# arkworks-rs/accumulation

Hardware: AMD Instinct MI355X
Metric: MSM throughput (point-scalar pairs/sec) at 2^20 Pallas (higher is better)
Workload: dtype u32; 1 GPU; 2^20-pair pallas MSM per GPU (north_star size; scalars uniform in [0, r), G_i = k_i*G), key resident + precomputed window multiples; pairs_per_gpu=1048576, curve=pallas, precomputed_key=True, parallelism=point-sharded x1, window_bits=20, pipeline=bucket-per-lane (k_prep_local_t + k_accum_bpl; skewed scalars re-run chunked), window_widths=9 x 20 + 4 x 19 bits = 256 (MsmGeom::n_narrow), msms_in_flight=3, full=False

## Files before the change

accumulation_amd/csrc/kern_fr.hip:

```cpp
#include "launch.h"
#include "vec_kernels.h"
#include "prep_kernels.h"

#include <algorithm>
#include <cmath>
#include <atomic>
#include <cstdlib>
#include <cstring>

namespace amsm {

static inline u32 cdiv_(u32 a, u32 b) { return (a + b - 1) / b; }
static u32 stream_grid(u32 n) {
  constexpr u32 per_cu = 64;
  static const u32 cus = [] {
    int dev = 0;
    hipDeviceProp_t prop;
    if (hipGetDevice(&dev) != hipSuccess || hipGetDeviceProperties(&prop, dev) != hipSuccess) return 256u;
    return (u32)std::max(1, prop.multiProcessorCount);
  }();
  return std::max(1u, std::min(cdiv_(n, 256), cus * per_cu));
}

void launch_bounds(hipStream_t st, const void* keys_sorted, bool keys16, u32* vals_sorted, MsmGeom g, u32* start,
                   u32* items) {
  if (keys16)
    hipLaunchKernelGGL((k_bounds<uint16_t>), dim3(cdiv_(g.B, 256)), dim3(256), 0, st, (const uint16_t*)keys_sorted,
                       vals_sorted, g, start, items);
  else
    hipLaunchKernelGGL((k_bounds<u32>), dim3(cdiv_(g.B, 256)), dim3(256), 0, st, (const u32*)keys_sorted, vals_sorted,
                       g, start, items);
}

constexpr u32 PREP_MAX_P = 4096;
static PrepGeom prep_geom(const MsmGeom& g) {
  PrepGeom pg;
  pg.SH = 4;
  while (((g.B + (1u << pg.SH) - 1u) >> pg.SH) > 512u && pg.SH < 10u) pg.SH++;
  while (((g.B + (1u << pg.SH) - 1u) >> pg.SH) > PREP_MAX_P) pg.SH++;
  pg.P = (g.B + (1u << pg.SH) - 1u) >> pg.SH;
  pg.SPB = g.S <= 16u ? 512u : 256u;
  unsigned long long max_idx = (unsigned long long)g.base_off + g.n - 1ull +
                               (g.precomp ? (unsigned long long)(g.W - 1u) * g.table_stride : 0ull);
  if (g.idx_rel_bits) max_idx = ((unsigned long long)(g.W - 1u) << g.idx_rel_bits) | ((1ull << g.idx_rel_bits) - 1ull);
  pg.IB = 1;
  while ((max_idx >> pg.IB) != 0ull) pg.IB++;
  while (pg.IB + pg.SH > 31u && pg.SH > 0u && ((g.B + (1u << (pg.SH - 1)) - 1u) >> (pg.SH - 1)) <= PREP_MAX_P) pg.SH--;
  pg.P = (g.B + (1u << pg.SH) - 1u) >> pg.SH;
  const u32 budget_words = 37888u, fixed_words = 2u * (1u << pg.SH) + 1024u;
  pg.CAP = budget_words > fixed_words + 4096u ? budget_words - fixed_words : 0u;
  pg.HEAVY = std::max<u32>(4u * (g.E / pg.P + 1u), 1u << 17);
  pg.FIX = 0;
  return pg;
}
static size_t prep_heavy_words(const MsmGeom& g) { return (size_t)g.B + 4096 + 64; }
size_t prep_small_words(const MsmGeom& g) { return 4 * (PREP_MAX_P + 1) + 1 + 3 * prep_heavy_words(g) + PREP_MAX_HEAVY; }
static size_t prep_local_lds(const PrepGeom& pg) { return (2 * (size_t)(1u << pg.SH) + 1024 + pg.CAP) * sizeof(u32); }
constexpr size_t PREP_LDS_LIMIT = 160 * 1024;
static std::atomic<unsigned long long> prep_local_attr_devices{0};
static void prep_local_attr() {
  int dev = 0;
  if (hipGetDevice(&dev) != hipSuccess || dev < 0 || dev >= 64) dev = 63;
  const unsigned long long bit = 1ull << dev;
  if (dev != 63 && (prep_local_attr_devices.load(std::memory_order_acquire) & bit)) return;
  (void)hipFuncSetAttribute((const void*)k_prep_local, hipFuncAttributeMaxDynamicSharedMemorySize, 152 * 1024);
  prep_local_attr_devices.fetch_or(bit, std::memory_order_release);
}
static size_t prep_scatter_lds(const MsmGeom& g, const PrepGeom& pg) {
  const size_t cap = (size_t)pg.SPB * g.S;
  return (3 * (size_t)pg.P + cap) * sizeof(u32) + cap * sizeof(uint16_t);
}
bool prep_supported(const MsmGeom& g) {
  if (g.n == 0 || g.S > 32u) return false;
  PrepGeom pg = prep_geom(g);
  return pg.SH <= 12u && pg.IB + pg.SH <= 31u && prep_scatter_lds(g, pg) <= PREP_LDS_LIMIT &&
         prep_local_lds(pg) <= PREP_LDS_LIMIT && (pg.P + 256) * sizeof(u32) <= 64 * 1024;
}

constexpr u32 BPL_LOCAL_FIXED_WORDS = 3u * BPL_NB + 2u * BPL_BINS + 2u * BPL_GROUPS + 2u;
constexpr u32 BPL_LOCAL_BUDGET_WORDS = 40960u;
static PrepGeom prep_bpl_geom(const MsmGeom& g) {
  PrepGeom pg;
  pg.SH = 10;
  pg.P = g.B >> pg.SH;
  pg.SPB = g.S <= 16u ? 512u : 256u;
  unsigned long long max_idx = (unsigned long long)g.base_off + g.n - 1ull +
                               (g.precomp ? (unsigned long long)(g.W - 1u) * g.table_stride : 0ull);
  if (g.idx_rel_bits) max_idx = ((unsigned long long)(g.W - 1u) << g.idx_rel_bits) | ((1ull << g.idx_rel_bits) - 1ull);
  pg.IB = 1;
  while ((max_idx >> pg.IB) != 0ull) pg.IB++;
  pg.CAP = BPL_LOCAL_BUDGET_WORDS - BPL_LOCAL_FIXED_WORDS;
  pg.HEAVY = 0xffffffffu;
  const unsigned long long per = std::max<unsigned long long>(((unsigned long long)g.E + pg.P - 1) / std::max(1u, pg.P), g.part_max);
  pg.FIX = (u32)std::min<unsigned long long>(pg.CAP, (per + per / 4ull + 2048ull + 15ull) & ~15ull);
  return pg;
}
size_t prep_bpl_part_entries(const MsmGeom& g) {
  PrepGeom pg = prep_bpl_geom(g);
  return std::max<size_t>(g.E, pg.FIX ? (size_t)pg.P * pg.FIX : 0);
}
static size_t prep_bpl_local_lds(const PrepGeom& pg) { return (size_t)(BPL_LOCAL_FIXED_WORDS + pg.CAP) * sizeof(u32); }
static size_t prep_bpl_scatter_lds(const MsmGeom& g, const PrepGeom& pg) {
  const size_t cap = (size_t)pg.SPB * g.S;
  return (3 * (size_t)pg.P + 2 * cap) * sizeof(u32) + cap * sizeof(uint16_t);
}
u32 prep_bpl_partitions(const MsmGeom& g) { return g.B >> 10; }
u32 prep_bpl_groups_per_partition() { return BPL_GROUPS; }
u32 prep_bpl_stride(const MsmGeom& g) {
  const u32 P = std::max(1u, prep_bpl_partitions(g));
  const unsigned long long per = std::max<unsigned long long>(((unsigned long long)g.E + P - 1) / P, g.part_max);
  return (u32)((per + per / 4ull + 4096ull + 1023ull) & ~1023ull);
}
bool prep_bpl_supported(const MsmGeom& g) {
  if (g.S > 32u || g.n == 0 || g.n_sets != g.groups * sets_per_group(g)) return false;
  if (g.B < (1u << 16) || (g.B & 1023u) || (g.B >> 10) > PREP_MAX_P || ((g.B >> 10) & 3u)) return false;
  PrepGeom pg = prep_bpl_geom(g);
  if (pg.IB > 30u) return false;
  if ((unsigned long long)g.E / pg.P + 1024ull > pg.CAP) return false;
  if (g.part_max && (unsigned long long)g.part_max + 5ull * (unsigned long long)std::sqrt((double)g.part_max) > pg.CAP) return false;
  return prep_bpl_scatter_lds(g, pg) <= PREP_LDS_LIMIT && prep_bpl_local_lds(pg) <= PREP_LDS_LIMIT &&
         (unsigned long long)pg.P * prep_bpl_stride(g) < (1ull << 31);
}
static std::atomic<unsigned long long> prep_bpl_attr_devices{0};
template <class KS>
static void prep_bpl_attr(KS scatter_kernel) {
  int dev = 0;
  if (hipGetDevice(&dev) != hipSuccess || dev < 0 || dev >= 64) dev = 63;
  const unsigned long long bit = 1ull << dev;
  (void)hipFuncSetAttribute((const void*)scatter_kernel, hipFuncAttributeMaxDynamicSharedMemorySize, (int)PREP_LDS_LIMIT);
  if (dev != 63 && (prep_bpl_attr_devices.load(std::memory_order_acquire) & bit)) return;
  static_assert((BPL_LOCAL_BUDGET_WORDS) * sizeof(u32) <= PREP_LDS_LIMIT, "k_prep_local_t's LDS must fit a workgroup");
  (void)hipFuncSetAttribute((const void*)k_prep_local_t, hipFuncAttributeMaxDynamicSharedMemorySize, (int)PREP_LDS_LIMIT);
  prep_bpl_attr_devices.fetch_or(bit, std::memory_order_release);
}

constexpr u32 bps_local_fixed_words(u32 nbp) { return 4u * nbp + 1024u + BPL_BINS + 2u * BPS_GROUPS + 2u; }
constexpr u32 BPS_LOCAL_BUDGET_WORDS = 37888u;
static PrepGeom prep_bps_geom(const MsmGeom& g, u32 log2_l) {
  PrepGeom pg;
  pg.SH = 10u - log2_l;
  pg.P = g.B >> pg.SH;
  pg.SPB = g.S <= 16u ? 512u : 256u;
  unsigned long long max_idx = (unsigned long long)g.base_off + g.n - 1ull +
                               (g.precomp ? (unsigned long long)(g.W - 1u) * g.table_stride : 0ull);
  if (g.idx_rel_bits) max_idx = ((unsigned long long)(g.W - 1u) << g.idx_rel_bits) | ((1ull << g.idx_rel_bits) - 1ull);
  pg.IB = 1;
  while ((max_idx >> pg.IB) != 0ull) pg.IB++;
  pg.CAP = BPS_LOCAL_BUDGET_WORDS - bps_local_fixed_words(1u << pg.SH);
  pg.HEAVY = 0xffffffffu;
  const unsigned long long per = ((unsigned long long)g.E + pg.P - 1) / std::max(1u, pg.P);
  pg.FIX = (u32)std::min<unsigned long long>(pg.CAP, (per + per / 2ull + 1024ull + 15ull) & ~15ull);
  return pg;
}
size_t prep_bps_part_entries(const MsmGeom& g, u32 log2_l) {
  PrepGeom pg = prep_bps_geom(g, log2_l);
  return std::max<size_t>(g.E, pg.FIX ? (size_t)pg.P * pg.FIX : 0);
}
static size_t prep_bps_local_lds(const PrepGeom& pg) {
  return (size_t)(bps_local_fixed_words(1u << pg.SH) + pg.CAP) * sizeof(u32);
}
u32 prep_bps_partitions(const MsmGeom& g, u32 log2_l) { return g.B >> (10u - log2_l); }
u32 prep_bps_stride(const MsmGeom& g, u32 log2_l) {
  const u32 P = std::max(1u, prep_bps_partitions(g, log2_l));
  const unsigned long long per = ((unsigned long long)g.E + P - 1) / P;
  return (u32)((per + per / 2ull + 4096ull + 1023ull) & ~1023ull);
}
int prep_bps_choose(const MsmGeom& g) {
  if (!g.precomp || g.n == 0 || g.S > 32u || g.B < 64u || (g.B & (g.B - 1u))) return -1;
  unsigned long long want = 128;
  while (want * 24576ull < g.E) want <<= 1;
  for (int l = 0; l <= 6; l++) {
    if ((10 - l) < 0 || (g.B >> (10 - l)) == 0) continue;
    const unsigned long long P = g.B >> (10 - l);
    if (P < want && l < 6) continue;
    if (P > PREP_MAX_P || (P & 1ull)) return -1;
    MsmGeom g2 = g;
    PrepGeom pg = prep_bps_geom(g2, (u32)l);
    if (pg.IB + pg.SH > 31u) return -1;
    if ((unsigned long long)g.E / P + 1024ull > pg.CAP) return -1;
    if (prep_scatter_lds(g, pg) > PREP_LDS_LIMIT || prep_bps_local_lds(pg) > PREP_LDS_LIMIT) return -1;
    if (P * (unsigned long long)prep_bps_stride(g, (u32)l) >= (1ull << 31)) return -1;
    return l;
  }
  return -1;
}
constexpr size_t PREP_BPS_ZERO_BYTES = (((16 + 4 * (PREP_MAX_P + 1) + 1) * sizeof(u32)) + 255) & ~(size_t)255;
u32 prep_bps_small_block_words() { return (u32)(PREP_BPS_ZERO_BYTES / sizeof(u32)); }
static std::atomic<unsigned long long> prep_bps_attr_devices{0};
static void prep_bps_attr() {
  int dev = 0;
  if (hipGetDevice(&dev) != hipSuccess || dev < 0 || dev >= 64) dev = 63;
  const unsigned long long bit = 1ull << dev;
  if (dev != 63 && (prep_bps_attr_devices.load(std::memory_order_acquire) & bit)) return;
  static_assert(BPS_LOCAL_BUDGET_WORDS * sizeof(u32) <= 152 * 1024, "k_prep_local_s's LDS must fit its attribute");
  (void)hipFuncSetAttribute((const void*)k_prep_local_s, hipFuncAttributeMaxDynamicSharedMemorySize, 152 * 1024);
  (void)hipFuncSetAttribute((const void*)k_prep_local_s_batch, hipFuncAttributeMaxDynamicSharedMemorySize, 152 * 1024);
  prep_bps_attr_devices.fetch_or(bit, std::memory_order_release);
}

__global__ void k_mirror_flags(const u32* __restrict__ flags, u32* __restrict__ host_mirror) {
  if (threadIdx.x < 2u) host_mirror[threadIdx.x] = flags[threadIdx.x];
}
void launch_mirror_flags(hipStream_t st, const u32* flags, u32* host_mirror) {
  hipLaunchKernelGGL(k_mirror_flags, dim3(1), dim3(64), 0, st, flags, host_mirror);
}
void launch_vec_fill(hipStream_t st, u32* out, const u32 v[8], u32 n) {
  hipLaunchKernelGGL(k_vec_fill, dim3(cdiv_(n, 256)), dim3(256), 0, st, out, make_uint4(v[0], v[1], v[2], v[3]),
                     make_uint4(v[4], v[5], v[6], v[7]), n);
}

void launch_tv_probe(hipStream_t st, const u32* scalars, u32 n, u32* out16, const u32 one[8]) {
  static_assert(TV_PROBE_WORDS == TV_WORDS && TV_EXC_SLOTS == TV_EXC_MAX && TV_ONES_SAMPLE_COUNT == TV_ONES_SAMPLES,
                "launch.h mirrors vec_kernels.h");
  const u32 blocks = std::max(1u, std::min(512u, (n + 1023u) / 1024u));
  TvOne o;
  memcpy(o.w, one, 32);
  hipLaunchKernelGGL(k_tv_probe, dim3(blocks), dim3(256), 0, st, scalars, n, out16, o);
}

#define AMSM_FR_LAUNCHERS(FR)                                                                                        \
  template <>                                                                                                        \
  int launch_prep<FR>(hipStream_t st, const u32* scalars, int mont, MsmGeom g, const PrepBuffers& b) {               \
    PrepGeom pg = prep_geom(g);                                                                                      \
    prep_local_attr();                                                                                               \
    u32* part_total = b.d_small;                                                                                     \
    u32* part_start = b.d_small + (PREP_MAX_P + 1);                                                                  \
    u32* part_cursor = b.d_small + 2 * (PREP_MAX_P + 1);                                                             \
    u32* part_items = b.d_small + 3 * (PREP_MAX_P + 1);                                                              \
    PrepHeavy hv;                                                                                                    \
    hv.n = b.d_small + 4 * (PREP_MAX_P + 1);                                                                         \
    hv.cnt = hv.n + 1;                                                          \
    hv.ids = hv.cnt + prep_heavy_words(g);                                                                           \
    hv.cur = hv.ids + PREP_MAX_HEAVY;                                                                                \
    hv.end = hv.cur + prep_heavy_words(g);                                                                           \
     \
     \
                                                                      \
    {                                                                                                                \
      size_t zero_bytes = (16 + 4 * (PREP_MAX_P + 1) + 1 + prep_heavy_words(g)) * sizeof(u32);                       \
      zero_bytes = (zero_bytes + 255) & ~(size_t)255;                                                                \
      if (b.err != b.d_small - 16) return -1;                                                                        \
      if (hipMemsetAsync(b.err, 0, zero_bytes, st) != hipSuccess) return -1;                                         \
    }                                                                                                                \
    u32 blocks = cdiv_(g.n, pg.SPB);                                                                                 \
    size_t lds_scatter = prep_scatter_lds(g, pg);                                                                    \
    if (lds_scatter > 64 * 1024) {                 \
      if (g.S <= 16u)                                                                                                \
        (void)hipFuncSetAttribute((const void*)k_prep_scatter<FR, 16, 1>, hipFuncAttributeMaxDynamicSharedMemorySize, \
                                  (int)PREP_LDS_LIMIT);                                                              \
      else                                                                                                           \
        (void)hipFuncSetAttribute((const void*)k_prep_scatter<FR, 32, 1>, hipFuncAttributeMaxDynamicSharedMemorySize, \
                                  (int)PREP_LDS_LIMIT);                                                              \
    }                                                                                                                \
    {                      \
      PrepGeom ph = pg;                                                                                              \
      ph.SPB = 1024;                                                                                                 \
      hipLaunchKernelGGL((k_prep_hist<FR>), dim3(cdiv_(g.n, 1024)), dim3(1024), pg.P * sizeof(u32), st, scalars,      \
                         mont, g, ph, part_total, b.err);                                                            \
    }                                                                                                                \
    hipLaunchKernelGGL(k_prep_scan, dim3(1), dim3(1024), 0, st, part_total, part_start, pg.P, pg.HEAVY, hv);         \
    if (g.S <= 16u)                                                                                                  \
      hipLaunchKernelGGL((k_prep_scatter<FR, 16, 1>), dim3(blocks), dim3(512), lds_scatter, st, scalars, mont, g, pg, \
                         part_start, part_cursor, b.part);                                                           \
    else                                                                                                             \
      hipLaunchKernelGGL((k_prep_scatter<FR, 32, 1>), dim3(blocks), dim3(256), lds_scatter, st, scalars, mont, g, pg, \
                         part_start, part_cursor, b.part);                                                           \
    const size_t lds_heavy = 2 * (size_t)(1u << pg.SH) * sizeof(u32);                                                \
    if (pg.HEAVY != 0xffffffffu)                                                                                     \
      hipLaunchKernelGGL(k_prep_heavy_count, dim3(PREP_HEAVY_GRID), dim3(256), lds_heavy, st, part_start, b.part, pg, hv); \
    hipLaunchKernelGGL(k_prep_local, dim3(pg.P), dim3(1024), prep_local_lds(pg), st,                                 \
                       part_start, b.part, g, pg, b.vals_sorted, b.start, b.items, b.item_off, part_items, hv);      \
    if (pg.HEAVY != 0xffffffffu)                                                                                     \
      hipLaunchKernelGGL(k_prep_heavy_place, dim3(PREP_HEAVY_GRID), dim3(256), lds_heavy, st, part_start, b.part, g, pg, hv, \
                         b.vals_sorted);                                                                             \
    hipLaunchKernelGGL(k_prep_offsets, dim3(cdiv_(g.B, 256)), dim3(256), (pg.P + 256) * sizeof(u32), st, part_start, \
                       part_items, pg, g, b.start, b.items, b.item_off, b.vals_sorted);                              \
    return 0;                                                                                                        \
  }                                                                                                                  \
  template <>                                                                                                        \
  int launch_prep_bps<FR>(hipStream_t st, const u32* scalars, int mont, MsmGeom g, u32 log2_l, const PrepBplBuffers& b) { \
    PrepGeom pg = prep_bps_geom(g, log2_l);                                                                          \
    u32* part_total = b.d_small;                                                                                     \
    u32* part_start = b.d_small + (PREP_MAX_P + 1);                                                                  \
    u32* part_cursor = b.d_small + 2 * (PREP_MAX_P + 1);                                                             \
    PrepHeavy hv;                                                                                                    \
    hv.n = b.d_small + 4 * (PREP_MAX_P + 1);                                                                         \
    hv.cnt = hv.n + 1;                                                                                               \
    hv.ids = hv.cnt + 64;                                                                                            \
    hv.cur = hv.end = hv.ids;                                                                                        \
    {                                                                                                                \
      size_t zero_bytes = (16 + 4 * (PREP_MAX_P + 1) + 1) * sizeof(u32);                                             \
      zero_bytes = (zero_bytes + 255) & ~(size_t)255;                                                                \
      if (b.err != b.d_small - 16) return -1;                                                                        \
      if (hipMemsetAsync(b.err, 0, zero_bytes, st) != hipSuccess) return -1;                                         \
    }                                                                                                                \
    prep_bps_attr();                                                                                                 \
    if (!pg.FIX) {                                                                                                   \
      PrepGeom ph = pg;                                                                                              \
      ph.SPB = 1024;                                                                                                 \
      hipLaunchKernelGGL((k_prep_hist<FR>), dim3(cdiv_(g.n, 1024)), dim3(1024), pg.P * sizeof(u32), st, scalars,      \
                         mont, g, ph, part_total, b.err);                                                            \
      hipLaunchKernelGGL(k_prep_scan, dim3(1), dim3(1024), 0, st, part_total, part_start, pg.P, pg.HEAVY, hv);       \
    }                                                                                                                \
    const size_t lds_scatter = prep_scatter_lds(g, pg);                                                              \
    if (g.S <= 16u) {                                                                                                \
      if (lds_scatter > 64 * 1024)                                                                                   \
        (void)hipFuncSetAttribute((const void*)k_prep_scatter<FR, 16, 1>, hipFuncAttributeMaxDynamicSharedMemorySize, \
                                  (int)PREP_LDS_LIMIT);                                                              \
      hipLaunchKernelGGL((k_prep_scatter<FR, 16, 1>), dim3(cdiv_(g.n, pg.SPB)), dim3(512), lds_scatter, st, scalars, \
                         mont, g, pg, part_start, part_cursor, b.part, b.err);                                       \
    } else {                                                                                                         \
      if (lds_scatter > 64 * 1024)                                                                                   \
        (void)hipFuncSetAttribute((const void*)k_prep_scatter<FR, 32, 1>, hipFuncAttributeMaxDynamicSharedMemorySize, \
                                  (int)PREP_LDS_LIMIT);                                                              \
      hipLaunchKernelGGL((k_prep_scatter<FR, 32, 1>), dim3(cdiv_(g.n, pg.SPB)), dim3(256), lds_scatter, st, scalars, \
                         mont, g, pg, part_start, part_cursor, b.part, b.err);                                       \
    }                                                                                                                \
    hipLaunchKernelGGL(k_prep_local_s, dim3(pg.P), dim3(1024), prep_bps_local_lds(pg), st,                           \
                       pg.FIX ? part_cursor : part_start, b.part, g, pg,                                             \
                       prep_bps_stride(g, log2_l), log2_l, b.ents_t, (BplGroup*)b.grp, b.order, b.err);              \
    return 0;                                                                                                        \
  }                                                                                                                  \
  template <>                                                                                                        \
  int launch_prep_bps_batch<FR>(hipStream_t st, const u32* const* scalars, u32 nv, int mont, MsmGeom g, u32 log2_l,   \
                                const BpsBatchBuffers& b) {                                                          \
    PrepGeom pg = prep_bps_geom(g, log2_l);                                                                          \
    const u32 stride = prep_bps_stride(g, log2_l);                                                                   \
                                  \
     \
     \
    if (nv < 1u || nv > (u32)PREP_BPS_BATCH || !pg.FIX || g.S > 16u || b.small_stride < prep_bps_small_block_words() || \
        (b.small_stride & 63u) || b.part_stride < prep_bps_part_entries(g, log2_l) ||                                \
        (unsigned long long)b.ents_stride < (unsigned long long)pg.P * stride || b.grp_stride < pg.P * BPS_GROUPS ||  \
        b.order_stride < g.B)                                                                                        \
      return -1;                                                                                                     \
    BpsBatchScalars sc;                                                                                              \
    for (u32 v = 0; v < (u32)PREP_BPS_BATCH; v++) sc.scalars[v] = scalars[v < nv ? v : 0u];                          \
    u32* part_start0 = b.small + 16 + (PREP_MAX_P + 1);                                                              \
    u32* part_cursor0 = b.small + 16 + 2 * (PREP_MAX_P + 1);                                                         \
                                                         \
    if (hipMemsetAsync(b.small, 0, (size_t)nv * b.small_stride * sizeof(u32), st) != hipSuccess) return -1;          \
    prep_bps_attr();                                                                                                 \
    const size_t lds_scatter = prep_scatter_lds(g, pg);                                                              \
    if (lds_scatter > 64 * 1024)                                                                                     \
      (void)hipFuncSetAttribute((const void*)k_prep_scatter_batch<FR, 16, 1>, hipFuncAttributeMaxDynamicSharedMemorySize, \
                                (int)PREP_LDS_LIMIT);                                                                \
    hipLaunchKernelGGL((k_prep_scatter_batch<FR, 16, 1>), dim3(cdiv_(g.n, pg.SPB), nv), dim3(512), lds_scatter, st, sc, mont, g,   \
                       pg, part_start0, part_cursor0, b.small_stride, b.part, b.part_stride, b.small);               \
    hipLaunchKernelGGL(k_prep_local_s_batch, dim3(pg.P, nv), dim3(1024), prep_bps_local_lds(pg), st, part_cursor0,   \
                       b.small_stride, b.part, b.part_stride, g, pg, stride, log2_l, b.ents_t, b.ents_stride,        \
                       (BplGroup*)b.grp, b.grp_stride, b.order, b.order_stride, b.small);                            \
    return 0;                                                                                                        \
  }                                                                                                                  \
  template <>                                                                                                        \
  int launch_prep_bpl<FR>(hipStream_t st, const u32* scalars, int mont, MsmGeom g, const PrepBplBuffers& b) {        \
    PrepGeom pg = prep_bpl_geom(g);                                                                                  \
    u32* part_total = b.d_small;                                                                                     \
    u32* part_start = b.d_small + (PREP_MAX_P + 1);                                                                  \
    u32* part_cursor = b.d_small + 2 * (PREP_MAX_P + 1);                                                             \
    PrepHeavy hv;                                                                                                    \
    hv.n = b.d_small + 4 * (PREP_MAX_P + 1);                                                                         \
    hv.cnt = hv.n + 1;                                                                                               \
    hv.ids = hv.cnt + 64;                                  \
    hv.cur = hv.end = hv.ids;                                                                                        \
    {                  \
      size_t zero_bytes = (16 + 4 * (PREP_MAX_P + 1) + 1) * sizeof(u32);                                             \
      zero_bytes = (zero_bytes + 255) & ~(size_t)255;                                                                \
      if (b.err != b.d_small - 16) return -1;                                                                        \
      if (hipMemsetAsync(b.err, 0, zero_bytes, st) != hipSuccess) return -1;                                         \
    }                                                                                                                \
    if (g.S <= 16u) prep_bpl_attr(k_prep_scatter<FR, 16, 1, true>);                                                  \
    else prep_bpl_attr(k_prep_scatter<FR, 32, 1, true>);                                                             \
    if (!pg.FIX) {                                                                                                   \
      PrepGeom ph = pg;                                                                                              \
      ph.SPB = 1024;                                                                                                 \
      hipLaunchKernelGGL((k_prep_hist<FR>), dim3(cdiv_(g.n, 1024)), dim3(1024), pg.P * sizeof(u32), st, scalars,      \
                         mont, g, ph, part_total, b.err);                                                            \
      hipLaunchKernelGGL(k_prep_scan, dim3(1), dim3(1024), 0, st, part_total, part_start, pg.P, pg.HEAVY, hv);       \
    }                                                                                                                \
    if (g.S <= 16u)                                                                                                  \
      hipLaunchKernelGGL((k_prep_scatter<FR, 16, 1, true>), dim3(cdiv_(g.n, pg.SPB)), dim3(512),                     \
                         prep_bpl_scatter_lds(g, pg), st, scalars, mont, g, pg, part_start, part_cursor, b.part, b.err); \
    else                                             \
// ... 132 lines not shown
```

accumulation_amd/csrc/prep_kernels.h:

```cpp
#pragma once
#include "fp.h"
#include "msm_select.h"
#include "msm_types.h"
#include "vec_kernels.h"

namespace amsm {

struct PrepGeom {
  u32 SH;
  u32 P;
  u32 SPB;
  u32 IB;
  u32 CAP;
  u32 HEAVY;
  u32 FIX;
};

constexpr u32 PREP_HEAVY_SLICES = 64, PREP_HEAVY_GRID = 1024, PREP_MAX_HEAVY = 4096;
struct PrepHeavy {
  u32* n;
  u32* ids;
  u32* cnt;
  u32* cur;
  u32* end;
// ... 170 lines not shown
          rsv_base[q] = pg.FIX ? p * pg.FIX : part_start[p];
          rsv[q] = atomicAdd(&part_cursor[p], v);
        }
        run += v;
      }
    }
    for (u32 p = lo + RSV_MAX; p < hi; p++) {
      u32 v = cnt[p];
      loff[p] = run;
      gbase[p] = v ? (pg.FIX ? p * pg.FIX : part_start[p]) + atomicAdd(&part_cursor[p], v) : 0u;
      run += v;
    }
  }
  __syncthreads();
  const u32 low = (1u << pg.SH) - 1u;
#pragma unroll
  for (int r = 0; r < SPT; r++) {
    u32 i = blockIdx.x * pg.SPB + r * T + t;
    if (i < g.n)
      scalar_entries_unrolled_reg<Fr, MAXW>(sreg[r], g, i, [&](int w, u32 key, u32 val) {
        u32 p = key >> pg.SH;
        u32 rank = (rk[r][w >> 1] >> ((w & 1) * 16)) & 0xffffu;
        u32 slot = loff[p] + rank;
        if (WIDE) reinterpret_cast<u64*>(staged)[slot] = ((u64)(key & low) << 32) | val;
        else staged[slot] = (val & 0x80000000u) | ((key & low) << pg.IB) | (val & 0x7fffffffu);
        staged_p[slot] = (uint16_t)p;
      });
  }
#pragma unroll
  for (u32 q = 0; q < RSV_MAX; q++)
    if (lo + q < hi) gbase[lo + q] = rsv_base[q] + rsv[q];
  __syncthreads();
  u32 total = loff[pg.P - 1] + cnt[pg.P - 1];
  for (u32 j = t; j < total; j += T) {
    u32 p = staged_p[j];
    const u32 dst = gbase[p] + (j - loff[p]);
    if (pg.FIX && dst - p * pg.FIX >= pg.FIX) continue;
    if (WIDE) reinterpret_cast<u64*>(part)[dst] = reinterpret_cast<const u64*>(staged)[j];
    else part[dst] = staged[j];
  }
}
template <class Fr, int MAXW, int SPT, bool WIDE = false>
__global__ void __launch_bounds__(512)
    k_prep_scatter(const u32* __restrict__ scalars, int mont, MsmGeom g, PrepGeom pg, const u32* __restrict__ part_start,
                   u32* __restrict__ part_cursor, u32* __restrict__ part, u32* __restrict__ err = nullptr) {
  prep_scatter_body<Fr, MAXW, SPT, WIDE>(scalars, mont, g, pg, part_start, part_cursor, part, err);
}
constexpr int PREP_BPS_BATCH = msel::BPS_BATCH;
struct BpsBatchScalars {
  const u32* scalars[PREP_BPS_BATCH];
};
template <class Fr, int MAXW, int SPT>
__global__ void __launch_bounds__(512)
    k_prep_scatter_batch(BpsBatchScalars b, int mont, MsmGeom g, PrepGeom pg, const u32* __restrict__ part_start0,
                         u32* __restrict__ part_cursor0, u32 small_stride, u32* __restrict__ part0, u32 part_stride,
                         u32* __restrict__ err) {
  const size_t v = blockIdx.y;
  prep_scatter_body<Fr, MAXW, SPT, false>(b.scalars[v], mont, g, pg, part_start0 + v * small_stride, part_cursor0 + v * small_stride,
                                          part0 + v * part_stride, err);
}

__global__ void __launch_bounds__(1024)
    k_prep_local(const u32* __restrict__ part_start, const u32* __restrict__ part, MsmGeom g, PrepGeom pg,
                 u32* __restrict__ vals_sorted, u32* __restrict__ start, u32* __restrict__ items, u32* __restrict__ item_off,
                 u32* __restrict__ part_items, PrepHeavy hv) {
  extern __shared__ u32 prep_lds[];
  const u32 NB = 1u << pg.SH;
  u32* cnt = prep_lds;
  u32* off = prep_lds + NB;
  u32* sl = prep_lds + 2 * NB;
  const u32 p = blockIdx.x, t = threadIdx.x, T = blockDim.x;
  const u32 ps = part_start[p], pe = part_start[p + 1];
  const u32 low = NB - 1u, idx_mask = (1u << pg.IB) - 1u;
  const bool heavy = (pe - ps) > pg.HEAVY;
  for (u32 k = t; k < NB; k += T) cnt[k] = heavy ? hv.cnt[(p << pg.SH) + k] : 0u;
  __syncthreads();
  const u32 body_lo = min((ps + 3u) & ~3u, pe), body_hi = max(body_lo, pe & ~3u);
  const bool skew = (pe - ps) > 4u * (g.E / pg.P + 1u);
  auto count = [&](u32 e) {
    u32 k = (e >> pg.IB) & low;
    if (skew) lds_count(cnt, k);
    else atomicAdd(&cnt[k], 1u);
  };
  if (!heavy) {
    for (u32 j = ps + t; j < body_lo; j += T) count(part[j]);
    for (u32 j = body_lo + 4u * t; j < body_hi; j += 4u * T) {
      uint4 e4 = *reinterpret_cast<const uint4*>(part + j);
      count(e4.x);
      count(e4.y);
      count(e4.z);
      count(e4.w);
    }
    for (u32 j = body_hi + t; j < pe; j += T) count(part[j]);
  }
  __syncthreads();
  const u32 b0 = p << pg.SH;
  u32 per = (NB + T - 1) / T;
  u32 lo_k = min(t * per, NB), hi_k = min(lo_k + per, NB);
  u32 sum = 0;
  for (u32 k = lo_k; k < hi_k; k++) sum += cnt[k];
  sl[t] = sum;
  __syncthreads();
  for (u32 d = 1; d < T; d <<= 1) {
    u32 v = t >= d ? sl[t - d] : 0u;
    __syncthreads();
    sl[t] += v;
    __syncthreads();
  }
  u32 run = sl[t] - sum;
  u32 my_items = 0;
  for (u32 k = lo_k; k < hi_k; k++) {
    u32 c = cnt[k];
    off[k] = run;
    u32 lo = ps + run, hi = lo + c;
    u32 it = c ? chunk_of(g, hi - 1) - chunk_of(g, lo) + 1 : 0u;
    if (b0 + k < g.B) {
      start[b0 + k] = lo;
      items[b0 + k] = it;
    }
    cnt[k] = run + c;
    if (heavy) {
      hv.cur[b0 + k] = run;
      hv.end[b0 + k] = run + c;
    }
    my_items += it;
    run += c;
  }
  __syncthreads();
  sl[t] = my_items;
  __syncthreads();
  for (u32 d = 1; d < T; d <<= 1) {
    u32 v = t >= d ? sl[t - d] : 0u;
    __syncthreads();
    sl[t] += v;
    __syncthreads();
  }
  u32 irun = sl[t] - my_items;
  for (u32 k = lo_k; k < hi_k; k++) {
    if (b0 + k < g.B) {
      item_off[b0 + k] = irun;
      irun += items[b0 + k];
    }
  }
  if (t == T - 1) part_items[p] = sl[T - 1];
  if (heavy) return;
  __syncthreads();
  u32* stage = prep_lds + 2 * NB + T;
  const bool staged = (pe - ps) <= pg.CAP;
  auto place = [&](u32 e) {
    u32 k = (e >> pg.IB) & low;
    u32 pos = skew ? lds_count(off, k) : atomicAdd(&off[k], 1u);
    u32 v = (e & 0x80000000u) | entry_abs_index(g, e & idx_mask);
    if (pos + 1 == cnt[k]) v |= PREP_ENTRY_LAST;
    if (staged) stage[pos] = v;
    else vals_sorted[ps + pos] = v;
  };
  for (u32 j = ps + t; j < body_lo; j += T) place(part[j]);
  for (u32 j = body_lo + 4u * t; j < body_hi; j += 4u * T) {
    uint4 e4 = *reinterpret_cast<const uint4*>(part + j);
    place(e4.x);
    place(e4.y);
    place(e4.z);
    place(e4.w);
  }
  for (u32 j = body_hi + t; j < pe; j += T) place(part[j]);
  if (staged) {
    __syncthreads();
    const u32 n_p = pe - ps;
    const u32 o_lo = min((ps + 3u) & ~3u, pe), o_hi = max(o_lo, pe & ~3u);
    for (u32 j = ps + t; j < o_lo; j += T) vals_sorted[j] = stage[j - ps];
    for (u32 j = o_lo + 4u * t; j < o_hi; j += 4u * T) {
      u32 q = j - ps;
      *reinterpret_cast<uint4*>(vals_sorted + j) = make_uint4(stage[q], stage[q + 1], stage[q + 2], stage[q + 3]);
    }
    for (u32 j = o_hi + t; j < pe; j += T) vals_sorted[j] = stage[j - ps];
    (void)n_p;
  }
}

AMSM_DEV void prep_heavy_slice(u32 ps, u32 pe, u32 s, u32& lo, u32& hi) {
  u32 per = ((pe - ps) + PREP_HEAVY_SLICES - 1u) / PREP_HEAVY_SLICES;
  lo = min(ps + s * per, pe);
  hi = min(lo + per, pe);
}
__global__ void __launch_bounds__(256)
    k_prep_heavy_count(const u32* __restrict__ part_start, const u32* __restrict__ part, PrepGeom pg, PrepHeavy hv) {
  extern __shared__ u32 prep_lds[];
  const u32 NB = 1u << pg.SH, low = NB - 1u, t = threadIdx.x, T = blockDim.x;
  u32* cnt = prep_lds;
  const u32 work = *hv.n * PREP_HEAVY_SLICES;
  for (u32 w = blockIdx.x; w < work; w += gridDim.x) {
    const u32 p = hv.ids[w / PREP_HEAVY_SLICES];
    u32 lo, hi;
    prep_heavy_slice(part_start[p], part_start[p + 1], w % PREP_HEAVY_SLICES, lo, hi);
    for (u32 k = t; k < NB; k += T) cnt[k] = 0;
    __syncthreads();
    for (u32 j = lo + t; j < hi; j += T) lds_count(cnt, (part[j] >> pg.IB) & low);
    __syncthreads();
    for (u32 k = t; k < NB; k += T)
      if (cnt[k]) atomicAdd(&hv.cnt[(p << pg.SH) + k], cnt[k]);
    __syncthreads();
  }
}
__global__ void __launch_bounds__(256)
    k_prep_heavy_place(const u32* __restrict__ part_start, const u32* __restrict__ part, MsmGeom g, PrepGeom pg, PrepHeavy hv,
                       u32* __restrict__ vals_sorted) {
  extern __shared__ u32 prep_lds[];
  const u32 NB = 1u << pg.SH, low = NB - 1u, idx_mask = (1u << pg.IB) - 1u, t = threadIdx.x, T = blockDim.x;
  u32* cnt = prep_lds;
  u32* base = prep_lds + NB;
  const u32 work = *hv.n * PREP_HEAVY_SLICES;
  for (u32 w = blockIdx.x; w < work; w += gridDim.x) {
    const u32 p = hv.ids[w / PREP_HEAVY_SLICES], b0 = p << pg.SH;
    const u32 ps = part_start[p];
    u32 lo, hi;
    prep_heavy_slice(ps, part_start[p + 1], w % PREP_HEAVY_SLICES, lo, hi);
    for (u32 k = t; k < NB; k += T) cnt[k] = 0;
    __syncthreads();
    for (u32 j = lo + t; j < hi; j += T) lds_count(cnt, (part[j] >> pg.IB) & low);
    __syncthreads();
    for (u32 k = t; k < NB; k += T) {
      u32 c = cnt[k];
      base[k] = c ? atomicAdd(&hv.cur[b0 + k], c) : 0u;
      cnt[k] = 0;
    }
    __syncthreads();
    for (u32 j = lo + t; j < hi; j += T) {
      u32 e = part[j];
      u32 k = (e >> pg.IB) & low;
      u32 pos = base[k] + lds_count(cnt, k);
      u32 v = (e & 0x80000000u) | entry_abs_index(g, e & idx_mask);
      if (pos + 1 == hv.end[b0 + k]) v |= PREP_ENTRY_LAST;
      vals_sorted[ps + pos] = v;
    }
    __syncthreads();
  }
}

__global__ void __launch_bounds__(256)
    k_prep_offsets(const u32* __restrict__ part_start, const u32* __restrict__ part_items, PrepGeom pg, MsmGeom g,
                   u32* __restrict__ start, u32* __restrict__ items, u32* __restrict__ item_off, u32* __restrict__ vals_sorted) {
  extern __shared__ u32 prep_lds[];
  u32* pref = prep_lds;
  u32* sl = prep_lds + pg.P;
  const u32 t = threadIdx.x, T = blockDim.x;
  u32 per = (pg.P + T - 1) / T;
  u32 lo = min(t * per, pg.P), hi = min(lo + per, pg.P);
  u32 sum = 0;
  for (u32 p = lo; p < hi; p++) sum += part_items[p];
  sl[t] = sum;
  __syncthreads();
  for (u32 d = 1; d < T; d <<= 1) {
    u32 v = t >= d ? sl[t - d] : 0u;
    __syncthreads();
    sl[t] += v;
    __syncthreads();
  }
  u32 run = sl[t] - sum;
  for (u32 p = lo; p < hi; p++) {
    pref[p] = run;
    run += part_items[p];
  }
  __syncthreads();
  u32 b = blockIdx.x * T + t;
  if (b < g.B) item_off[b] += pref[b >> pg.SH];
  if (blockIdx.x == 0) {
    const u32 e_valid = part_start[pg.P];
    if (t == 0) {
      start[g.B] = e_valid;
      items[g.B] = 0;
      item_off[g.B] = sl[T - 1];
    }
    const u32 span = 256u * max(g.K0, g.K0b);
    unsigned long long reach = (unsigned long long)e_valid + span + 16ull;
    const u32 pad_end = (u32)min(reach, (unsigned long long)((g.E + 3u) & ~3u));
    for (u32 k = e_valid + t; k < pad_end; k += T) vals_sorted[k] = 0;
  }
}

constexpr u32 BPL_GROUP = 64;
constexpr u32 BPL_ENTRY_PAD = 0x40000000u;
constexpr u32 BPL_BINS = 256;
constexpr u32 BPL_SPLIT = 64;
constexpr u32 BPL_NB = 1024;
constexpr u32 BPL_LANES = BPL_NB + BPL_SPLIT;
constexpr u32 BPL_GROUPS = BPL_LANES / BPL_GROUP;
struct BplGroup {
  u32 base;
  u32 m;
};
AMSM_DEV void bpl_slot(u32 s, u32& pos, u32& half) {
  if (s < BPL_SPLIT) {
    pos = s >> 1;
    half = 1u + (s & 1u);
  } else if (s >= BPL_NB) {
    pos = BPL_SPLIT / 2u + ((s - BPL_NB) >> 1);
    half = 1u + (s & 1u);
  } else {
    pos = s;
    half = 0u;
  }
}

__global__ void __launch_bounds__(1024)
    k_prep_local_t(const u32* __restrict__ part_start, const u64* __restrict__ part, MsmGeom g, PrepGeom pg, u32 stride,
                   u32* __restrict__ ents_t, BplGroup* __restrict__ grp, u32* __restrict__ order, u32* __restrict__ err) {
  extern __shared__ u32 prep_lds[];
  const u32 NB = BPL_NB, NG = BPL_GROUPS;
  u32* cnt = prep_lds;
  u32* cur = cnt + NB;
  u32* ord = cur + NB;
  u32* bins = ord + NB;
  u32* bscan = bins + BPL_BINS;
  u32* gm = bscan + BPL_BINS;
  u32* gb = gm + NG;
  u32* stage = gb + NG + 1;
  u32* sl = stage;
  const u32 p = blockIdx.x, t = threadIdx.x, T = blockDim.x;
  const u32 ps = pg.FIX ? p * pg.FIX : part_start[p];
  const u32 n_p = pg.FIX ? part_start[p] : part_start[p + 1] - ps;
  const u32 pe = ps + (pg.FIX ? min(n_p, pg.FIX) : n_p);
  const u32 low = NB - 1u, idx_mask = (1u << pg.IB) - 1u, b0 = p << pg.SH;
  const bool fits = n_p <= pg.CAP && (!pg.FIX || n_p <= pg.FIX);
  for (u32 k = t; k < NB; k += T) cnt[k] = 0;
  for (u32 k = t; k < BPL_BINS; k += T) bins[k] = 0;
  for (u32 k = t; k < NG; k += T) gm[k] = 0;
  __syncthreads();
  if (fits)
    for (u32 j = ps + t; j < pe; j += T) atomicAdd(&cnt[(u32)(part[j] >> 32) & low], 1u);
  __syncthreads();
  const u32 c_t = t < NB ? cnt[t] : 0u;
  sl[t] = c_t;
  __syncthreads();
  for (u32 d = 1; d < T; d <<= 1) {
    u32 v = t >= d ? sl[t - d] : 0u;
    __syncthreads();
    sl[t] += v;
    __syncthreads();
  }
  if (t < NB) cur[t] = sl[t] - c_t;
  const u32 bin = min(c_t, BPL_BINS - 1u);
  u32 rank = 0;
  if (t < NB) rank = atomicAdd(&bins[bin], 1u);
  __syncthreads();
  if (fits)
    for (u32 j = ps + t; j < pe; j += T) {
      const u64 e = part[j];
      const u32 k = (u32)(e >> 32) & low, lo = (u32)e;
      const u32 pos = atomicAdd(&cur[k], 1u);
      stage[pos] = (lo & 0x80000000u) | entry_abs_index(g, lo & idx_mask);
    }
  if (t < BPL_BINS) bscan[t] = bins[BPL_BINS - 1u - t];
  __syncthreads();
  for (u32 d = 1; d < BPL_BINS; d <<= 1) {
    u32 v = (t < BPL_BINS && t >= d) ? bscan[t - d] : 0u;
    __syncthreads();
    if (t < BPL_BINS) bscan[t] += v;
    __syncthreads();
  }
  if (t < BPL_BINS) bins[BPL_BINS - 1u - t] = bscan[t] - bins[BPL_BINS - 1u - t];
  __syncthreads();
  u32 my_pos = 0;
  if (t < NB) {
    my_pos = bins[bin] + rank;
    ord[my_pos] = t;
    const u32 h0 = (c_t + 1u) >> 1;
    if (my_pos < BPL_SPLIT / 2u) atomicMax(&gm[0], h0);
    else if (my_pos < BPL_SPLIT) atomicMax(&gm[NG - 1u], h0);
    else atomicMax(&gm[my_pos / BPL_GROUP], c_t);
  }
  __syncthreads();
  if (t == 0) {
    u32 run = 0;
    for (u32 q = 0; q < NG; q++) {
      gb[q] = run;
      run += gm[q] * BPL_GROUP;
    }
    gb[NG] = run;
  }
  __syncthreads();
  const u32 total = gb[NG];
  const bool ok = fits && total <= stride;
  if (!ok && t == 0) atomicOr(err + 1, 1u);
  if (t < NG) {
    BplGroup h;
    h.base = p * stride + gb[t];
    h.m = ok ? gm[t] : 0u;
    grp[p * NG + t] = h;
  }
  if (t < NB) {
    u32* o = order + (size_t)p * BPL_LANES;
    if (my_pos < BPL_SPLIT / 2u) o[2u * my_pos] = o[2u * my_pos + 1u] = b0 + t;
    else if (my_pos < BPL_SPLIT) o[BPL_NB + 2u * (my_pos - BPL_SPLIT / 2u)] = o[BPL_NB + 2u * (my_pos - BPL_SPLIT / 2u) + 1u] = b0 + t;
    else o[my_pos] = b0 + t;
  }
  if (!ok) return;
  for (u32 j = t; j < total; j += T) {
    u32 q = 0;
    while (q + 1u < NG && gb[q + 1u] <= j) q++;
    const u32 k = (j - gb[q]) / BPL_GROUP, l = j % BPL_GROUP;
    u32 pos, half;
    bpl_slot(q * BPL_GROUP + l, pos, half);
    const u32 kb = ord[pos], c = cnt[kb], h0 = (c + 1u) >> 1;
    const u32 off = half == 2u ? h0 : 0u, sz = half == 0u ? c : (half == 1u ? h0 : c - h0);
    ents_t[(size_t)p * stride + j] = k < sz ? stage[cur[kb] - c + off + k] : BPL_ENTRY_PAD;
  }
}

constexpr u32 BPS_LANES = 1024, BPS_GROUPS = BPS_LANES / BPL_GROUP;
AMSM_DEV void prep_local_s_body(const u32* part_start, const u32* part, MsmGeom g, PrepGeom pg, u32 stride, u32 log2_l, u32* ents_t,
                                BplGroup* grp, u32* order, u32* err) {
  extern __shared__ u32 prep_lds[];
  const u32 NBP = 1u << pg.SH, L = 1u << log2_l, NG = BPS_GROUPS;
  u32* cnt = prep_lds;
  u32* cur = cnt + NBP;
  u32* beg = cur + NBP;
  u32* ord = beg + NBP;
  u32* sl = ord + NBP;
  u32* bins = sl + 1024;
  u32* gm = bins + BPL_BINS;
  u32* gb = gm + NG;
  u32* stage = gb + NG + 2;
  const u32 p = blockIdx.x, t = threadIdx.x, T = blockDim.x;
  const u32 ps = pg.FIX ? p * pg.FIX : part_start[p];
  const u32 n_p = pg.FIX ? part_start[p] : part_start[p + 1] - ps;
  const u32 pe = ps + (pg.FIX ? min(n_p, pg.FIX) : n_p);
  const u32 low = NBP - 1u, idx_mask = (1u << pg.IB) - 1u;
  const bool fits = n_p <= pg.CAP && (!pg.FIX || n_p <= pg.FIX);
  for (u32 k = t; k < NBP; k += T) cnt[k] = 0;
  for (u32 k = t; k < BPL_BINS; k += T) bins[k] = 0;
  for (u32 k = t; k < NG; k += T) gm[k] = 0;
  __syncthreads();
  if (fits)
    for (u32 j = ps + t; j < pe; j += T) atomicAdd(&cnt[(part[j] >> pg.IB) & low], 1u);
  __syncthreads();
  const u32 c_t = t < NBP ? cnt[t] : 0u;
  sl[t] = c_t;
  __syncthreads();
  for (u32 d = 1; d < T; d <<= 1) {
    u32 v = t >= d ? sl[t - d] : 0u;
    __syncthreads();
    sl[t] += v;
    __syncthreads();
  }
  if (t < NBP) {
    beg[t] = sl[t] - c_t;
    cur[t] = sl[t] - c_t;
  }
  const u32 bin = min(c_t, BPL_BINS - 1u);
  u32 rank = 0;
  if (t < NBP) rank = atomicAdd(&bins[bin], 1u);
  __syncthreads();
  if (fits)
    for (u32 j = ps + t; j < pe; j += T) {
      const u32 e = part[j];
      const u32 pos = atomicAdd(&cur[(e >> pg.IB) & low], 1u);
      stage[pos] = (e & 0x80000000u) | entry_abs_index(g, e & idx_mask);
    }
  if (t < BPL_BINS) sl[t] = bins[BPL_BINS - 1u - t];
  __syncthreads();
  for (u32 d = 1; d < BPL_BINS; d <<= 1) {
    u32 v = (t < BPL_BINS && t >= d) ? sl[t - d] : 0u;
    __syncthreads();
    if (t < BPL_BINS) sl[t] += v;
    __syncthreads();
  }
  if (t < BPL_BINS) bins[BPL_BINS - 1u - t] = sl[t] - bins[BPL_BINS - 1u - t];
  __syncthreads();
  if (t < NBP) {
    const u32 my_pos = bins[bin] + rank;
    ord[my_pos] = t;
    order[(size_t)p * NBP + my_pos] = p * NBP + t;
    atomicMax(&gm[(my_pos << log2_l) / BPL_GROUP], (c_t + L - 1u) >> log2_l);
  }
  __syncthreads();
  if (t == 0) {
    u32 run = 0;
    for (u32 q = 0; q < NG; q++) {
      gb[q] = run;
      run += gm[q] * BPL_GROUP;
    }
    gb[NG] = run;
  }
  __syncthreads();
  const u32 total = gb[NG];
  const bool ok = fits && total <= stride;
  if (!ok && t == 0) atomicOr(err + 1, 1u);
  if (t < NG) {
    BplGroup h;
    h.base = p * stride + gb[t];
    h.m = ok ? gm[t] : 0u;
    grp[p * NG + t] = h;
  }
  if (!ok) return;
  for (u32 j = t; j < total; j += T) {
    u32 q = 0;
    while (q + 1u < NG && gb[q + 1u] <= j) q++;
    const u32 k = (j - gb[q]) / BPL_GROUP, l = j % BPL_GROUP;
    const u32 lane = q * BPL_GROUP + l, kb = ord[lane >> log2_l], r = lane & (L - 1u);
    const u32 i = (k << log2_l) + r;
    ents_t[(size_t)p * stride + j] = i < cnt[kb] ? stage[beg[kb] + i] : BPL_ENTRY_PAD;
  }
}
__global__ void __launch_bounds__(1024)
    k_prep_local_s(const u32* __restrict__ part_start, const u32* __restrict__ part, MsmGeom g, PrepGeom pg, u32 stride,
                   u32 log2_l, u32* __restrict__ ents_t, BplGroup* __restrict__ grp, u32* __restrict__ order,
                   u32* __restrict__ err) {
  prep_local_s_body(part_start, part, g, pg, stride, log2_l, ents_t, grp, order, err);
}
__global__ void __launch_bounds__(1024)
    k_prep_local_s_batch(const u32* __restrict__ part_cursor0, u32 small_stride, const u32* __restrict__ part0, u32 part_stride,
                         MsmGeom g, PrepGeom pg, u32 stride, u32 log2_l, u32* __restrict__ ents0, u32 ents_stride,
                         BplGroup* __restrict__ grp0, u32 grp_stride, u32* __restrict__ order0, u32 order_stride,
                         u32* __restrict__ err) {
  const size_t v = blockIdx.y;
  prep_local_s_body(part_cursor0 + v * small_stride, part0 + v * part_stride, g, pg, stride, log2_l, ents0 + v * ents_stride,
                    grp0 + v * grp_stride, order0 + v * order_stride, err);
}

}
```

Baseline: 988.6 million pairs/s.

## Keep partition entries in registers and use wave-shuffle scans in k_prep_local_t

The prep kernel now loads each partition's entries once into per-lane register slots (37 u64 per thread) and reuses them for both the counting pass and the scatter pass, rather than reading global memory twice. The LDS Hillis-Steele scans, which needed a barrier per step, are replaced by a wave-shuffle inclusive scan with a small cross-wave combine. The serial group-base loop and the per-element group search in the output loop are replaced by per-wave row striding over the groups. The cost is heavy register pressure at 1024 threads, which could cause spills, and the atomics are now batched per slot block.

```diff
diff --git a/accumulation_amd/csrc/kern_fr.hip b/accumulation_amd/csrc/kern_fr.hip
--- a/accumulation_amd/csrc/kern_fr.hip
+++ b/accumulation_amd/csrc/kern_fr.hip
@@ -79,6 +79,8 @@
 
 constexpr u32 BPL_LOCAL_FIXED_WORDS = 3u * BPL_NB + 2u * BPL_BINS + 2u * BPL_GROUPS + 2u;
 constexpr u32 BPL_LOCAL_BUDGET_WORDS = 40960u;
+static_assert(BPL_LOCAL_BUDGET_WORDS - BPL_LOCAL_FIXED_WORDS <= BPL_LOCAL_SLOTS * BPL_NB,
+              "k_prep_local_t keeps a partition of CAP entries in BPL_LOCAL_SLOTS registers per lane");
 static PrepGeom prep_bpl_geom(const MsmGeom& g) {
   PrepGeom pg;
   pg.SH = 10;
diff --git a/accumulation_amd/csrc/prep_kernels.h b/accumulation_amd/csrc/prep_kernels.h
--- a/accumulation_amd/csrc/prep_kernels.h
+++ b/accumulation_amd/csrc/prep_kernels.h
@@ -496,108 +496,144 @@
   }
 }
 
+AMSM_DEV u32 block_scan_inclusive(u32 v, u32* wt) {
+  const u32 lane = __lane_id(), w = threadIdx.x >> 6;
+#pragma unroll
+  for (u32 d = 1; d < 64u; d <<= 1) {
+    const u32 o = __shfl_up(v, d);
+    if (lane >= d) v += o;
+  }
+  if (lane == 63u) wt[w] = v;
+  __syncthreads();
+  u32 before = 0;
+#pragma unroll
+  for (u32 i = 0; i < 15u; i++) before += i < w ? wt[i] : 0u;
+  return v + before;
+}
+
+constexpr u32 BPL_LOCAL_SLOTS = 37, BPL_SLOT_BLOCK = 8;
+template <class F>
+AMSM_DEV void bpl_slot_blocks(u32 n, F&& f) {
+#pragma unroll
+  for (u32 b = 0; b < BPL_LOCAL_SLOTS; b += BPL_SLOT_BLOCK)
+    if (b * BPL_NB < n) f(b);
+}
+
 __global__ void __launch_bounds__(1024)
     k_prep_local_t(const u32* __restrict__ part_start, const u64* __restrict__ part, MsmGeom g, PrepGeom pg, u32 stride,
                    u32* __restrict__ ents_t, BplGroup* __restrict__ grp, u32* __restrict__ order, u32* __restrict__ err) {
   extern __shared__ u32 prep_lds[];
-  const u32 NB = BPL_NB, NG = BPL_GROUPS;
+  constexpr u32 NB = BPL_NB, NG = BPL_GROUPS, T = BPL_NB, SLOTS = BPL_LOCAL_SLOTS, BLK = BPL_SLOT_BLOCK;
   u32* cnt = prep_lds;
   u32* cur = cnt + NB;
-  u32* ord = cur + NB;
-  u32* bins = ord + NB;
-  u32* bscan = bins + BPL_BINS;
-  u32* gm = bscan + BPL_BINS;
-  u32* gb = gm + NG;
-  u32* stage = gb + NG + 1;
-  u32* sl = stage;
-  const u32 p = blockIdx.x, t = threadIdx.x, T = blockDim.x;
+  u32* wt = cur + NB;
+  u32* bins = wt + NB;
+  u32* first = bins + BPL_BINS;
+  u32* gm = first + BPL_BINS;
+  u32* stage = gm + 2u * NG + 1u;
+  const u32 p = blockIdx.x, t = threadIdx.x;
   const u32 ps = pg.FIX ? p * pg.FIX : part_start[p];
   const u32 n_p = pg.FIX ? part_start[p] : part_start[p + 1] - ps;
   const u32 pe = ps + (pg.FIX ? min(n_p, pg.FIX) : n_p);
   const u32 low = NB - 1u, idx_mask = (1u << pg.IB) - 1u, b0 = p << pg.SH;
   const bool fits = n_p <= pg.CAP && (!pg.FIX || n_p <= pg.FIX);
-  for (u32 k = t; k < NB; k += T) cnt[k] = 0;
-  for (u32 k = t; k < BPL_BINS; k += T) bins[k] = 0;
-  for (u32 k = t; k < NG; k += T) gm[k] = 0;
-  __syncthreads();
-  if (fits)
-    for (u32 j = ps + t; j < pe; j += T) atomicAdd(&cnt[(u32)(part[j] >> 32) & low], 1u);
-  __syncthreads();
-  const u32 c_t = t < NB ? cnt[t] : 0u;
-  sl[t] = c_t;
-  __syncthreads();
-  for (u32 d = 1; d < T; d <<= 1) {
-    u32 v = t >= d ? sl[t - d] : 0u;
-    __syncthreads();
-    sl[t] += v;
-    __syncthreads();
-  }
-  if (t < NB) cur[t] = sl[t] - c_t;
+  const u32 n = fits ? min(pe - ps, SLOTS * T) : 0u;
+  u64 e[SLOTS];
+#pragma unroll
+  for (u32 i = 0; i < SLOTS; i++) e[i] = 0;
+  bpl_slot_blocks(n, [&](u32 b) {
+#pragma unroll
+    for (u32 i = b; i < b + BLK && i < SLOTS; i++) e[i] = part[ps + min(i * T + t, n - 1u)];
+  });
+  cnt[t] = 0;
+  if (t < BPL_BINS) bins[t] = 0;
+  if (t < NG) gm[t] = 0;
+  __syncthreads();
+  bpl_slot_blocks(n, [&](u32 b) {
+#pragma unroll
+    for (u32 i = b; i < b + BLK && i < SLOTS; i++)
+      if (i * T + t < n) atomicAdd(&cnt[(u32)(e[i] >> 32) & low], 1u);
+  });
+  __syncthreads();
+  const u32 c_t = cnt[t];
+  const u32 first_t = block_scan_inclusive(c_t, wt) - c_t;
+  cur[t] = first_t;
   const u32 bin = min(c_t, BPL_BINS - 1u);
-  u32 rank = 0;
-  if (t < NB) rank = atomicAdd(&bins[bin], 1u);
-  __syncthreads();
-  if (fits)
-    for (u32 j = ps + t; j < pe; j += T) {
-      const u64 e = part[j];
-      const u32 k = (u32)(e >> 32) & low, lo = (u32)e;
-      const u32 pos = atomicAdd(&cur[k], 1u);
-      stage[pos] = (lo & 0x80000000u) | entry_abs_index(g, lo & idx_mask);
-    }
-  if (t < BPL_BINS) bscan[t] = bins[BPL_BINS - 1u - t];
-  __syncthreads();
-  for (u32 d = 1; d < BPL_BINS; d <<= 1) {
-    u32 v = (t < BPL_BINS && t >= d) ? bscan[t - d] : 0u;
-    __syncthreads();
-    if (t < BPL_BINS) bscan[t] += v;
-    __syncthreads();
-  }
-  if (t < BPL_BINS) bins[BPL_BINS - 1u - t] = bscan[t] - bins[BPL_BINS - 1u - t];
-  __syncthreads();
-  u32 my_pos = 0;
-  if (t < NB) {
-    my_pos = bins[bin] + rank;
-    ord[my_pos] = t;
+  const u32 rank = atomicAdd(&bins[bin], 1u);
+  __syncthreads();
+  bpl_slot_blocks(n, [&](u32 b) {
+    u32 pos[BLK];
+#pragma unroll
+    for (u32 i = b; i < b + BLK && i < SLOTS; i++) {
+      pos[i - b] = 0;
+      if (i * T + t < n) pos[i - b] = atomicAdd(&cur[(u32)(e[i] >> 32) & low], 1u);
+    }
+#pragma unroll
+    for (u32 i = b; i < b + BLK && i < SLOTS; i++) {
+      const u32 lo = (u32)e[i];
+      if (i * T + t < n) stage[pos[i - b]] = (lo & 0x80000000u) | entry_abs_index(g, lo & idx_mask);
+    }
+  });
+  const u32 in_class = t < BPL_BINS ? bins[BPL_BINS - 1u - t] : 0u;
+  const u32 larger = block_scan_inclusive(in_class, wt + 16) - in_class;
+  if (t < BPL_BINS) first[BPL_BINS - 1u - t] = larger;
+  __syncthreads();
+  const u32 my_pos = first[bin] + rank;
+  cnt[my_pos] = c_t;
+  cur[my_pos] = first_t;
+  {
     const u32 h0 = (c_t + 1u) >> 1;
     if (my_pos < BPL_SPLIT / 2u) atomicMax(&gm[0], h0);
     else if (my_pos < BPL_SPLIT) atomicMax(&gm[NG - 1u], h0);
     else atomicMax(&gm[my_pos / BPL_GROUP], c_t);
   }
   __syncthreads();
-  if (t == 0) {
-    u32 run = 0;
-    for (u32 q = 0; q < NG; q++) {
-      gb[q] = run;
-      run += gm[q] * BPL_GROUP;
-    }
-    gb[NG] = run;
-  }
-  __syncthreads();
-  const u32 total = gb[NG];
+  u32 total = 0, my_gb = 0;
+#pragma unroll
+  for (u32 q = 0; q < NG; q++) {
+    if (q == t) my_gb = total;
+    total += gm[q] * BPL_GROUP;
+  }
   const bool ok = fits && total <= stride;
   if (!ok && t == 0) atomicOr(err + 1, 1u);
   if (t < NG) {
     BplGroup h;
-    h.base = p * stride + gb[t];
+    h.base = p * stride + my_gb;
     h.m = ok ? gm[t] : 0u;
     grp[p * NG + t] = h;
   }
-  if (t < NB) {
+  {
     u32* o = order + (size_t)p * BPL_LANES;
     if (my_pos < BPL_SPLIT / 2u) o[2u * my_pos] = o[2u * my_pos + 1u] = b0 + t;
     else if (my_pos < BPL_SPLIT) o[BPL_NB + 2u * (my_pos - BPL_SPLIT / 2u)] = o[BPL_NB + 2u * (my_pos - BPL_SPLIT / 2u) + 1u] = b0 + t;
     else o[my_pos] = b0 + t;
   }
   if (!ok) return;
-  for (u32 j = t; j < total; j += T) {
-    u32 q = 0;
-    while (q + 1u < NG && gb[q + 1u] <= j) q++;
-    const u32 k = (j - gb[q]) / BPL_GROUP, l = j % BPL_GROUP;
+  const u32 w = t >> 6, l = t & 63u;
+  auto slot_of = [&](u32 q, u32& sz, u32& src) {
     u32 pos, half;
     bpl_slot(q * BPL_GROUP + l, pos, half);
-    const u32 kb = ord[pos], c = cnt[kb], h0 = (c + 1u) >> 1;
-    const u32 off = half == 2u ? h0 : 0u, sz = half == 0u ? c : (half == 1u ? h0 : c - h0);
-    ents_t[(size_t)p * stride + j] = k < sz ? stage[cur[kb] - c + off + k] : BPL_ENTRY_PAD;
+    const u32 c = cnt[pos], h0 = (c + 1u) >> 1;
+    sz = half == 0u ? c : (half == 1u ? h0 : c - h0);
+    src = cur[pos] + (half == 2u ? h0 : 0u);
+  };
+  u32* out = ents_t + (size_t)p * stride + l;
+  u32 row0 = 0, sz, src, m = gm[0];
+  slot_of(0, sz, src);
+  for (u32 q = 0; q < NG; q++) {
+    u32 sz_n = 0, src_n = 0, m_n = 0;
+    if (q + 1u < NG) {
+      m_n = gm[q + 1u];
+      slot_of(q + 1u, sz_n, src_n);
+    }
+    for (u32 k = (w - row0) & 15u; k < m; k += 16u) {
+      const u32 v = stage[k < sz ? src + k : 0u];
+      out[(size_t)(row0 + k) * BPL_GROUP] = k < sz ? v : BPL_ENTRY_PAD;
+    }
+    row0 += m;
+    sz = sz_n;
+    src = src_n;
+    m = m_n;
   }
 }
 
```

Result: faster. 1.011 billion pairs/s (median of 6 runs) (+2.3%).
